# jmhb0/view_neti

Hardware: AMD Instinct MI355X
Metric: TI train steps/sec (SD-1.5 512^2 bs=4 per GPU) (higher is better)
Workload: dtype f16; 1 GPU; learnable_mode 0, sd15 shapes, 512x512 fp16, bs=4/GPU, grad_accum 1, full train step (VAE+16xCLIP+UNet fwd/bwd+AdamW); global_batch=4, parallelism=dp1, rccl_ranks=1, hipgraph=True

## Files before the change

include/vneti.h:

```cpp
#ifndef VNETI_H
#define VNETI_H
#include <stddef.h>
#include <stdint.h>

#ifdef __cplusplus
extern "C" {
#endif

#define VNETI_ABI_VERSION 1

int vneti_version(void);
int vneti_precision(void);
int vneti_last_error(char* buf, size_t n);

typedef struct vneti_gemm_desc {
  const void* A;
  const void* B;
  void* C;
  long long lda, ldb, ldc;
  int M, N, K;
  int batch;
  long long strideA, strideB, strideC;
  const float* bias;
  const void* rowadd;
// ... 1 lines not shown
  int rows_per_group;
  const void* resid;
  long long ldr;
  float alpha;
  int act;
  int out_f32;
  int conv_mode;
  int Hi, Wi, Ci, Ho, Wo, stride, pad_t, pad_l, ups;
  long long ldx;
  int tile_hint;
  void* workspace;
  long long workspace_bytes;
  int split_k;
  const void* gate_src;
  long long ld_gate;
  int gate_act;
  void* C2;
  long long ldc2;
  int act2;
  void* gn_sums;
  int gn_hw, gn_cpg, gn_groups, gn_slots;
  int geglu;
  int conv_korder;
} vneti_gemm_desc;

int vneti_gemm_f16(const vneti_gemm_desc* d, void* stream);
int vneti_gemm_select_tile(int M, int N, int batch);
int vneti_gemm_select_split(int M, int N, int K, int batch, int tile_hint, long long workspace_bytes);

int vneti_im2col3x3_small(const void* x, int x_is_f32, long long sb, long long sc, long long sy,
                          long long sx, void* out, int Bn, int C, int Hi, int Wi, int Ho, int Wo,
                          int stride, int pad_t, int pad_l, void* stream);

int vneti_conv3x3_in(const void* x, int x_is_f32, long long sb, long long sc, long long sy, long long sx,
                     const void* w_packed, const float* bias, void* out, long long ldo, int Bn, int C, int H, int W,
                     int Co, void* gn_sums, int gn_groups, int gn_slots, void* stream);

int vneti_transpose_f16(const void* in, long long ld_in, long long stride_in, void* out,
                        long long ld_out, long long stride_out, int rows, int cols, int batch,
                        void* stream);
#define VNETI_TRANSPOSE_MAX 4
typedef struct vneti_transpose_desc {
  const void* inp;
  long long ld_in, stride_in;
  void* out;
  long long ld_out, stride_out;
// ... 227 lines not shown
```

view_neti_amd/csrc/gemm_args.h:

```cpp
#pragma once
#include "common.h"

namespace {

struct GemmArgs {
  const half_t* A;
  const half_t* B;
  void* C;
  const float* bias;
  const half_t* rowadd;
  const void* resid;
  float* ws;
  const half_t* gate_src;
  half_t* C2;
  long long ld_gate, ldc2;
  int gate_act, act2;
  float* gn_sums;
  int gn_hw, gn_cpg, gn_G, gn_slots;
  int geglu;
  long long lda, ldb, ldc, ld_rowadd, ldr;
  long long strideA, strideB, strideC;
  uint32_t a_bytes, b_bytes;
  int M, N, K;
  int rows_per_group;
  float alpha;
  int act;
  int out_f32;
  int batch, ksplit, kt_per_split;
  int conv_mode;
  int Hi, Wi, Ci, Ho, Wo, stride, pad_t, pad_l, ups;
  int ldx2;
  int korder;
  int tiles_m, tiles_n;
};

__device__ __forceinline__ float apply_act(float v, int act) {
  switch (act) {
    case 1: return vn_silu(v);
    case 2: return vn_quick_gelu(v);
    case 3: return vn_gelu_erf(v);
    default: return v;
  }
}
__device__ __forceinline__ float act_grad(float f, int act) {
  if (act == 2) {
    float s = vn_sigmoid(1.702f * f);
    return s * (1.f + 1.702f * f * (1.f - s));
  } else if (act == 3) {
    return vn_gelu_erf_grad(f);
  }
  float s = vn_sigmoid(f);
  return s * (1.f + f * (1.f - s));
}

__device__ __forceinline__ int lds_off(int row, int chunk) {
// ... 15 lines not shown
```

view_neti_amd/csrc/gemm_conv.hip:

```cpp
#include "common.h"
#include "gemm_args.h"
#include "../../include/vneti.h"

namespace {

template <int BM, int BN, int WM, int WN, bool F32OUT, bool DMA, int NSTG = 2, int EPI = 2, bool CONV = true>
__global__ __launch_bounds__((BM / WM) * (BN / WN) * 64) void gemm_kernel(
    const half_t* pA, const half_t* pB, uint32_t p_a_bytes, uint32_t p_b_bytes, int p_lda, int p_ldb, int pM, int pN, int pK,
    int p_tiles_m, int p_tiles_n, int p_split_conv , const GemmArgs gfull) {
  GemmArgs g = gfull;
  g.A = pA;
  g.B = pB;
  g.a_bytes = p_a_bytes;
  g.b_bytes = p_b_bytes;
  g.lda = p_lda;
  g.ldb = p_ldb;
  g.M = pM;
  g.N = pN;
  g.K = pK;
  g.tiles_m = p_tiles_m;
  g.tiles_n = p_tiles_n;
  g.kt_per_split = p_split_conv & 0xffff;
  g.ksplit = (p_split_conv >> 16) & 0xff;
  g.conv_mode = p_split_conv >> 24;
// ... 18 lines not shown
  __shared__ __attribute__((aligned(16))) char smem[LDS_BYTES + GN_BYTES];

  const int tid = threadIdx.x;
  const int lane = tid & 63;
  const int wave = __builtin_amdgcn_readfirstlane(tid >> 6);
  const int wm0 = (wave / NWN) * WM;
  const int wn0 = (wave % NWN) * WN;

  int nblk = g.tiles_m * g.tiles_n;
  int bid = blockIdx.x;
  {
    int q = nblk >> 3, r = nblk & 7, xcd = bid & 7, idx = bid >> 3;
    bid = (xcd < r ? xcd * (q + 1) : r * (q + 1) + (xcd - r) * q) + idx;
  }
  const int tile_m = bid / g.tiles_n;
  const int tile_n = bid - tile_m * g.tiles_n;
  const int m0 = tile_m * BM;
  const int n0 = tile_n * BN;
  const int bz = blockIdx.y;
  const int kz = blockIdx.z;

  const half_t* Ab = g.A + (long long)bz * g.strideA;
  const half_t* Bb = g.B + (long long)bz * g.strideB;
  __amdgpu_buffer_rsrc_t rsA = vn_make_rsrc(Ab, g.a_bytes);
  __amdgpu_buffer_rsrc_t rsB = vn_make_rsrc(Bb, g.b_bytes);

  const int lrow = tid >> 3;
  const int gchunk = DMA ? ((tid & 7) ^ ((lrow >> 1) & 7)) : (tid & 7);

  const float rcp_hw = CONV ? __builtin_amdgcn_rcpf((float)(g.Ho * g.Wo)) : 0.f, rcp_wo = CONV ? __builtin_amdgcn_rcpf((float)g.Wo) : 0.f;
  int a_off[A_IT];
  int a_py[A_IT], a_px[A_IT], a_bh[A_IT];
#pragma unroll
  for (int i = 0; i < A_IT; ++i) {
    int m = m0 + lrow + RSTEP * i;
    bool ok = m < g.M;
    if (e_conv == 0) {
      a_off[i] = ok ? (int)((long long)m * g.lda * 2) + gchunk * 16 : -1;
      a_py[i] = a_px[i] = a_bh[i] = 0;
    } else {
      int rem, ox;
      const int b = vn_divmod(m, g.Ho * g.Wo, rcp_hw, rem);
      const int oy = vn_divmod(rem, g.Wo, rcp_wo, ox);
      a_bh[i] = ok ? b * g.Hi : -1;
      if (e_conv == 1) {
        a_py[i] = oy * g.stride - g.pad_t;
        a_px[i] = ox * g.stride - g.pad_l;
      } else {
        a_py[i] = oy + g.pad_t;
        a_px[i] = ox + g.pad_l;
      }
      a_off[i] = ((b * g.Hi + a_py[i]) * g.Wi + a_px[i]) * g.ldx2 + gchunk * 16;
    }
  }
  int b_off[B_IT];
#pragma unroll
  for (int i = 0; i < B_IT; ++i) {
    int n = n0 + lrow + RSTEP * i;
    b_off[i] = (n < g.N) ? (int)((long long)n * g.ldb * 2) + gchunk * 16 : -1;
  }

  u32x4 ra[DMA ? 1 : A_IT], rb[DMA ? 1 : B_IT];

  auto a_offset = [&](int i, int k0, int dy, int dx, int tapoff) -> uint32_t {
    if (e_conv == 0) return a_off[i] < 0 ? VN_OOB : (uint32_t)(a_off[i] + k0 * 2);
    bool ok = a_bh[i] >= 0;
    if (e_conv == 1 && !g.ups) {
      int iy = a_py[i] + dy, ix = a_px[i] + dx;
      ok = ok && (unsigned)iy < (unsigned)g.Hi && (unsigned)ix < (unsigned)g.Wi;
      return ok ? (uint32_t)(a_off[i] + tapoff) : VN_OOB;
    }
    int iy, ix;
    if (e_conv == 1) {
      iy = a_py[i] + dy;
      ix = a_px[i] + dx;
      ok = ok && (unsigned)iy < (unsigned)(2 * g.Hi) && (unsigned)ix < (unsigned)(2 * g.Wi);
      iy >>= 1;
      ix >>= 1;
    } else {
      int ty = a_py[i] - dy, tx = a_px[i] - dx;
      ok = ok && ty >= 0 && tx >= 0;
      if (g.stride == 2) {
        ok = ok && ((ty | tx) & 1) == 0;
        ty >>= 1;
        tx >>= 1;
      }
      iy = ty;
      ix = tx;
      ok = ok && iy < g.Hi && ix < g.Wi;
    }
    return ok ? (uint32_t)(((a_bh[i] + iy) * g.Wi + ix) * g.ldx2 + tapoff) : VN_OOB;
  };

  uint32_t a_cur[A_IT], b_cur[B_IT];
#pragma unroll
  for (int i = 0; i < B_IT; ++i) b_cur[i] = b_off[i] < 0 ? VN_OOB : (uint32_t)b_off[i];

  auto issue = [&](int kt, int stage, bool first) {
    const int k0 = kt * 64;
    bool recompute = first;
    int dy = 0, dx = 0, tapoff = 0;
    if (e_conv != 0) {
      int tap, ci0;
      if (g.korder) {
        const int chunk = kt / 9;
        tap = kt - chunk * 9;
        ci0 = chunk << 6;
        recompute = true;
      } else {
        tap = k0 / g.Ci;
        ci0 = k0 - tap * g.Ci;
        recompute = recompute || ci0 == 0;
      }
      if (recompute) {
        dy = tap / 3;
        dx = tap - dy * 3;
        tapoff = (e_conv == 1 && !g.ups) ? ((dy * g.Wi + dx) * g.ldx2 + ci0 * 2) : (ci0 * 2 + gchunk * 16);
      }
    }
    if (recompute) {
#pragma unroll
      for (int i = 0; i < A_IT; ++i) a_cur[i] = a_offset(i, k0, dy, dx, tapoff);
      if (first) {
#pragma unroll
        for (int i = 0; i < B_IT; ++i) b_cur[i] += (uint32_t)k0 * 2;
      }
    }
    if constexpr (DMA) {
      char* As = smem + stage * STAGE_BYTES;
      char* Bs = As + BM * 128;
#pragma unroll
      for (int i = 0; i < A_IT; ++i) dma16(rsA, As + (wave * 8 + RSTEP * i) * 128, a_cur[i]);
#pragma unroll
      for (int i = 0; i < B_IT; ++i) dma16(rsB, Bs + (wave * 8 + RSTEP * i) * 128, b_cur[i]);
    } else {
#pragma unroll
      for (int i = 0; i < A_IT; ++i) ra[i] = vn_buf_load16(rsA, a_cur[i]);
#pragma unroll
      for (int i = 0; i < B_IT; ++i) rb[i] = vn_buf_load16(rsB, b_cur[i]);
    }
// ... 238 lines not shown
        }
      }
      if (gn_img >= 0 && (!uni || lane < CPR)) {
        vn_u64* a = gacc + ((gn_img - gn_img0) * GN_NG + (gn_glo - gn_g0t)) * 4;
        vn_fx_add2(a, s_lo, q_lo);
        if (gn_split < 8) vn_fx_add2(a + 4, s_hi, q_hi);
      }
      s_lo = q_lo = s_hi = q_hi = 0.f;
    };
    for (int idx = tid; idx < BM * CPR; idx += NT) {
      int r = idx / CPR, c = (idx - r * CPR) * 8;
      int m = m0 + r, n = n0 + c;
      const bool valid = m < g.M && n < g.N;
      if (gn) {
        int gn_rem;
        const int img = valid ? vn_divmod(m, g.gn_hw, rcp_gnhw, gn_rem) : gn_img;
        if (__any(img != gn_img)) {
          gn_flush();
          gn_img = img;
        }
      }
      if (!valid) continue;
      half8 v = as_half8(*reinterpret_cast<const u32x4*>(smem + ((size_t)r * CS_LD + c) * 2));
      int ra_rem;
      const half_t* radd = e_rowadd ? e_rowadd + (long long)vn_divmod(m, g.rows_per_group, rcp_rpg, ra_rem) * g.ld_rowadd + n : nullptr;
      if (n + 8 <= g.N) {
        if (radd) {
          half8 t = *reinterpret_cast<const half8*>(radd);
          v = vn_add8(v, t);
        }
        if (Rb) {
          half8 rr = *reinterpret_cast<const half8*>(Rb + (long long)m * g.ldr + n);
          v = vn_add8(v, rr);
        }
        if (e_geglu == 2) {
          const half_t* pp = e_gate + (long long)m * g.ld_gate + 2 * n;
#pragma unroll
          for (int c2 = 0; c2 < 2; ++c2) {
            const half8 pre = *reinterpret_cast<const half8*>(pp + 8 * c2);
            half8 o;
#pragma unroll
            for (int e = 0; e < 4; ++e) {
              const float d = (float)v[4 * c2 + e], hh = (float)pre[e], gg = (float)pre[4 + e];
              float cdf, xpdf;
              vn_gelu_parts(gg, cdf, xpdf);
              o[e] = (half_t)(d * gg * cdf);
              o[4 + e] = (half_t)(d * hh * (cdf + xpdf));
            }
            vn_st16_wt(rsC, (uint32_t)(((long long)m * g.ldc + 2 * n + 8 * c2) * 2), o);
          }
          continue;
        }
        if (e_gate) {
          half8 pre = *reinterpret_cast<const half8*>(e_gate + (long long)m * g.ld_gate + n);
#pragma unroll
          for (int e = 0; e < 8; ++e) v[e] = (half_t)((float)v[e] * act_grad((float)pre[e], g.gate_act));
        }
        if (e_geglu == 1 || (e_C2 && e_geglu == 0)) vn_st16_wt_saved(rsC, (uint32_t)(((long long)m * g.ldc + n) * 2), v);
        else vn_st16_wt(rsC, (uint32_t)(((long long)m * g.ldc + n) * 2), v);
        if (e_geglu == 1) {
          half4 o2;
#pragma unroll
          for (int e = 0; e < 4; ++e) o2[e] = (half_t)((float)v[e] * vn_gelu_erf((float)v[4 + e]));
          *reinterpret_cast<half4*>(e_C2 + (long long)m * g.ldc2 + (n >> 1)) = o2;
        }
        if (gn) {
#pragma unroll
          for (int e = 0; e < 8; ++e) {
            const float x = (float)v[e];
            if (e < gn_split) {
              s_lo += x;
              q_lo += x * x;
            } else {
              s_hi += x;
              q_hi += x * x;
            }
          }
        }
        if (e_C2 && e_geglu == 0) {
          half8 o2;
#pragma unroll
          for (int e = 0; e < 8; ++e) o2[e] = (half_t)apply_act((float)v[e], g.act2);
          vn_st16_wt(rsC2, (uint32_t)(((long long)m * g.ldc2 + n) * 2), o2);
        }
      } else {
        for (int e = 0; e < 8 && n + e < g.N; ++e) {
          float x = (float)v[e];
          if (radd) x = (float)(half_t)(x + (float)radd[e]);
          if (Rb) x = (float)(half_t)(x + (float)Rb[(long long)m * g.ldr + n + e]);
          if (e_gate) x = (float)(half_t)(x * act_grad((float)e_gate[(long long)m * g.ld_gate + n + e], g.gate_act));
          Cb[(long long)m * g.ldc + n + e] = (half_t)x;
          if (e_C2) e_C2[(long long)m * g.ldc2 + n + e] = (half_t)apply_act((float)(half_t)x, g.act2);
          if (gn) {
            const float xs = (float)(half_t)x;
            if (e < gn_split) {
              s_lo += xs;
              q_lo += xs * xs;
            } else {
              s_hi += xs;
              q_hi += xs * xs;
            }
          }
        }
      }
    }
    if (gn) {
      gn_flush();
      __syncthreads();
      const int slot = tile_m % g.gn_slots;
      for (int i = tid; i < GN_IMG * GN_NG; i += NT) {
        const vn_u64* src = gacc + 4 * i;
        if ((src[0] | src[1] | src[2] | src[3]) == 0) continue;
        const int img = gn_img0 + i / GN_NG, grp = gn_g0t + i % GN_NG;
        vn_u64* dst = reinterpret_cast<vn_u64*>(e_gn_sums) + (((long long)img * g.gn_slots + slot) * g.gn_G + grp) * 4;
// ... 244 lines not shown
  g.geglu = d->geglu;
  g.lda = d->lda;
  g.ldb = d->ldb;
  g.ldc = d->ldc;
  g.ld_rowadd = d->ld_rowadd;
  g.ldr = d->ldr;
  g.strideA = d->strideA;
  g.strideB = d->strideB;
  g.strideC = d->strideC;
  g.M = d->M;
  g.N = d->N;
  g.K = d->K;
  g.batch = batch;
  g.rows_per_group = d->rows_per_group > 0 ? d->rows_per_group : 1;
  g.alpha = d->alpha;
  g.act = d->act;
  g.out_f32 = d->out_f32 ? 1 : 0;
  g.conv_mode = d->conv_mode;
  long long a_bytes;
  if (d->conv_mode == 0) {
    VN_REQUIRE(d->lda % 8 == 0, "gemm: lda=%lld must be a multiple of 8", d->lda);
    a_bytes = ((long long)(d->M - 1) * d->lda + d->K) * 2;
  } else {
    VN_REQUIRE(d->conv_mode == 1 || d->conv_mode == 2, "gemm: bad conv_mode %d", d->conv_mode);
    VN_REQUIRE(d->Ci > 0 && d->Ci % 64 == 0, "conv: Ci=%d must be a multiple of 64", d->Ci);
    VN_REQUIRE(d->K == 9 * d->Ci, "conv: K=%d must equal 9*Ci=%d", d->K, 9 * d->Ci);
    VN_REQUIRE(d->stride == 1 || d->stride == 2, "conv: stride %d unsupported", d->stride);
    VN_REQUIRE(d->Ho > 0 && d->Wo > 0 && d->M % (d->Ho * d->Wo) == 0, "conv: M=%d not a multiple of Ho*Wo", d->M);
    VN_REQUIRE(d->ldx % 8 == 0, "conv: ldx must be a multiple of 8");
    VN_REQUIRE(!(d->ups && d->conv_mode != 1), "conv: fused upsample only in forward gather mode");
    VN_REQUIRE(!(d->ups && d->stride != 1), "conv: fused upsample needs stride 1");
    g.Hi = d->Hi;
    g.Wi = d->Wi;
    g.Ci = d->Ci;
    g.Ho = d->Ho;
    g.Wo = d->Wo;
    g.stride = d->stride;
    g.pad_t = d->pad_t;
    g.pad_l = d->pad_l;
    g.ups = d->ups;
    g.ldx2 = (int)(d->ldx * 2);
    VN_REQUIRE(!d->conv_korder || d->Ci % 64 == 0, "conv: conv_korder=1 needs Ci=%d to be a multiple of 64", d->Ci);
    g.korder = d->conv_korder ? 1 : 0;
    long long nb = d->M / (d->Ho * d->Wo);
    a_bytes = nb * d->Hi * d->Wi * d->ldx * 2;
  }
  long long b_bytes = ((long long)(d->N - 1) * d->ldb + d->K) * 2;
  VN_REQUIRE(a_bytes < 0x7fffffffLL && b_bytes < 0x7fffffffLL, "gemm: operand larger than 2 GiB");
  g.a_bytes = (uint32_t)a_bytes;
  g.b_bytes = (uint32_t)b_bytes;
  if (!d->out_f32) {
    VN_REQUIRE(d->ldc % 8 == 0 || d->N < 8, "gemm: ldc=%lld must be a multiple of 8", d->ldc);
  }
  VN_REQUIRE_OUT("gemm C", vn_out_bytes(d->M, d->ldc, d->N, d->out_f32 ? 4 : 2, batch, d->strideC));
  if (d->C2) VN_REQUIRE_OUT("gemm C2", vn_out_bytes(d->M, d->ldc2, d->geglu == 1 ? d->N / 2 : d->N, 2));
  hipStream_t st = (hipStream_t)stream;
  bool f32 = d->out_f32 != 0;
  VN_REQUIRE(!(f32 && d->rowadd), "gemm: rowadd is only supported for f16 output");
  if (d->gate_src || d->C2) {
    VN_REQUIRE(!f32 && batch == 1, "gemm: gate/C2 epilogues need f16 output and batch 1");
    VN_REQUIRE(!d->gate_src || (d->gate_act >= 1 && d->gate_act <= 3 && d->ld_gate % 8 == 0), "gemm: bad gate arguments");
    VN_REQUIRE(!d->C2 || (d->act2 >= 0 && d->act2 <= 3 && d->ldc2 % 8 == 0), "gemm: bad C2 arguments");
  }

  if (d->geglu) {
    VN_REQUIRE(d->geglu == 1 || d->geglu == 2, "gemm: geglu must be 0, 1 or 2");
    VN_REQUIRE(!f32 && batch == 1 && d->N % 8 == 0, "gemm: geglu needs f16 output, batch 1 and N %% 8 == 0");
    VN_REQUIRE(d->split_k == 1, "gemm: geglu needs split_k = 1 (it lives in the fused epilogue)");
    VN_REQUIRE(!d->gn_sums, "gemm: geglu and gn_sums are exclusive");
    if (d->geglu == 1) {
      VN_REQUIRE(d->C2 && d->ldc2 % 4 == 0 && !d->gate_src, "gemm: geglu forward needs C2 ([M][N/2]) and no gate");
    } else {
      VN_REQUIRE(d->gate_src && d->ld_gate % 8 == 0 && !d->C2 && !d->resid && !d->rowadd,
                 "gemm: geglu backward needs gate_src ([M][2N] saved pre-activation) and a plain epilogue");
      VN_REQUIRE(d->ldc % 8 == 0, "gemm: geglu backward writes [M][2N]: ldc %% 8");
    }
  }
  if (d->gn_sums) {
    VN_REQUIRE(!f32 && batch == 1, "gemm: gn_sums needs f16 output and batch 1");
    VN_REQUIRE(d->gn_hw >= 64 && d->gn_cpg >= 4 && d->gn_groups > 0 && d->gn_slots > 0 && d->N == d->gn_cpg * d->gn_groups &&
                   d->M % d->gn_hw == 0 && (d->gn_cpg >= 8 || d->gn_cpg == 4),
               "gemm: bad gn_sums geometry hw=%d cpg=%d G=%d", d->gn_hw, d->gn_cpg, d->gn_groups);
    VN_REQUIRE(d->split_k == 1, "gemm: gn_sums needs split_k = 1 (the statistics live in the fused epilogue)");
  }

  int cfg = d->tile_hint;
  bool dma = true;
  if (cfg >= 100) {
    dma = false;
    cfg -= 100;
  }
  if (cfg == 0) cfg = select_tile(d->M, d->N, batch);
  VN_REQUIRE(cfg >= 1 && cfg <= kMaxTile, "gemm: unknown tile_hint %d", d->tile_hint);
  if (cfg == 18 &&
      (d->conv_mode < 1 || d->conv_mode > 2 || d->stride != 1 || d->ups || d->pad_t != 1 || d->pad_l != 1 || d->Hi != d->Ho ||
       d->Wi != d->Wo || (d->Ho & 15) || (d->Wo & 15) || (d->Ci & 63) || !d->conv_korder || batch != 1 || f32))
    cfg = 17;
  if (cfg == 18 && d->gn_sums && (d->gn_cpg & 1)) cfg = 17;
  if ((cfg == 16 || cfg == 17) && (!dma || (d->conv_mode && (d->ups || (d->conv_mode == 2 && d->stride == 2))) ||
                    (d->gn_sums && (d->gn_cpg & 1)) ||
                    (d->M >= (1 << 24) && (d->conv_mode || d->rowadd || d->gn_sums)))) cfg = cfg == 16 ? 5 : 7;
  if ((cfg == 5 || cfg == 16) && f32) cfg = 4;
  if (cfg == 17 && f32) cfg = 7;
  if ((cfg == 6 || cfg == 7) && !dma) cfg = 4;
  if (cfg >= 10 && !dma) cfg = kTiles[cfg].bm == 128 ? (kTiles[cfg].bn == 128 ? 1 : 2) : 3;
  long long ws_floats = d->workspace ? d->workspace_bytes / 4 : 0;
  int ks = d->split_k;
  if (ks == 0) ks = select_ksplit(d->M, d->N, d->K, batch, cfg, ws_floats);
  if (ks < 1) ks = 1;
  const int nk = d->K / 64;
  if (ks > nk) ks = nk;
  if (ks > 1) {
    VN_REQUIRE(d->workspace && (long long)ks * batch * d->M * d->N <= ws_floats,
               "gemm: split_k=%d needs %lld workspace bytes", ks, (long long)ks * batch * d->M * d->N * 4);
    VN_REQUIRE(batch == 1 || (d->strideC != 0), "gemm: batched split-K needs strideC");
    VN_REQUIRE((long long)batch * d->M * ((d->N + 3) / 4) < 0x7fffffffLL, "gemm: split-K output larger than 2^31 chunks");
    VN_REQUIRE_OUT("gemm split-K workspace", (long long)ks * batch * d->M * d->N * 4);
  }
  if (cfg == 18 && ks > d->Ci / 64) ks = d->Ci / 64;
  g.ksplit = ks;
  g.kt_per_split = cdiv(nk, ks);
  g.ksplit = cdiv(nk, g.kt_per_split);
// ... 34 lines not shown
```

view_neti_amd/engine/schedule.py:

```python
from __future__ import annotations

from functools import partial
from typing import Dict, List

import torch

from .. import lib, ops, packing


class T:

    __slots__ = ("v", "g", "gw", "rows", "cols", "children", "need_grad", "producer")

    def __init__(self, v, g=None, need_grad=True):
        self.v = v
        self.g = g
        self.gw = False
        self.rows, self.cols = v.shape
        self.children: List["T"] = []
        self.need_grad = need_grad
        self.producer = None


def rup(x, m):
# ... 51 lines not shown
    def _grad(self, t: T):
        if t.g is None:
            t.g = self._buf((t.rows, t.cols))
        return t.g

    def _contrib(self, t: T, fn, extra=None):
        g = self._grad(t)
        if t.gw:
            if extra is not None:
                self.bwd.append(partial(ops.add, g, extra, g))
            self.bwd.append(self._tagged(partial(fn, g, g), fn))
        else:
            self.bwd.append(self._tagged(partial(fn, g, extra), fn))
            t.gw = True
            for c in t.children:
                c.gw = True

    @staticmethod
    def _tagged(p, fn):
        if hasattr(fn, "vn_cost"):
            p.vn_cost = fn.vn_cost
        return p

    def _contrib_gemm(self, t: T, A, Bm, **kw):
        g = self._grad(t)
        resid = g if t.gw else None
        self.bwd.append(partial(ops.gemm, A, Bm, g, resid=resid, **kw))
        if not t.gw:
            t.gw = True
            for c in t.children:
                c.gw = True

    _tile_cache: Dict[tuple, int] = {}
    _TILE_DIMS = {1: (128, 128), 2: (128, 64), 3: (64, 64), 4: (256, 128), 5: (256, 256), 6: (256, 128), 7: (256, 128),
                  8: (256, 128), 9: (128, 128), 10: (128, 128), 11: (128, 64), 12: (64, 64), 13: (128, 128), 14: (128, 64),
                  15: (64, 64), 16: (256, 256), 17: (256, 128), 18: (256, 128)}

    @staticmethod
    def _gemm_key(f):
        kw = f.keywords
        A, Bm, out = f.args[:3]
        conv = kw.get("conv")
        M = kw.get("M") or A.shape[-2]
        N = kw.get("N") or Bm.shape[-2]
        K = kw.get("K") or Bm.shape[-1]
        ck = (conv["mode"], conv["stride"], conv["ups"], conv["Hi"], conv["Wi"]) if conv else None
        return (M, N, K, kw.get("batch") or 1, ck, out.dtype == torch.float32, kw.get("geglu") or 0)

    def autotune(self, candidates=(1, 2, 3, 5, 6, 7, 8, 9, 10, 11, 12, 13, 14, 15, 16, 17, 18), reps=8):
        if not torch.cuda.is_available():
# ... 44 lines not shown
            t = _time_call(partial(ops.gemm, *args, **kw), args[0], *how)
            if t < best_t:
                best, best_t = (h, sk, ko), t
        return best, B_cm

    def _pin(self, f, pick, B_cm=None):
        pick = tuple(pick) + (0,) * (3 - len(pick))
        conv = f.keywords.get("conv")
        kw = dict(f.keywords)
        kw["tile_hint"], kw["split_k"] = pick[0], pick[1]
        args = f.args
        if pick[2] and _chunk_major_ok(conv):
            if B_cm is None:
                B_cm = packing._chunk_major(f.args[1], f.args[1].shape[0], conv["Ci"])
            kw["conv"] = dict(conv, korder=1)
            self.bytes += B_cm.numel() * B_cm.element_size()
            args = (f.args[0], B_cm) + tuple(f.args[2:])
        return partial(ops.gemm, *args, **kw)

    def bind_workspace(self):
        for lst in (self.fwd_pre, self.fwd, self.bwd):
            for idx, f in enumerate(lst):
                fn = getattr(f, "func", None)
                if fn is ops.gemm or fn is ops.attn_bwd_dkv:
                    lst[idx] = self._rebound(f, fn, dict(f.keywords, workspace=self.ws))

    @staticmethod
    def _rebound(f, fn, kw):
        return partial(fn, *f.args, **kw)

    GN_SLOTS = 8

    def _produced(self, t: T):
        t.producer = len(self.fwd) - 1
        return t

    GN2_MAX = 512

    def _gn2_slice(self):
        if not hasattr(self, "_gn2_arena"):
            self._gn2_arena = self._buf((self.GN2_MAX, self.B, self.GN_SLOTS, self.groups, 4), torch.int64, zero=True)
            self._gn2_used = 0
        assert self._gn2_used < self.GN2_MAX
        self._gn2_used += 1
        return self._gn2_arena[self._gn2_used - 1]

    def fuse_gn_stats(self, fuse: bool = True):
# ... 146 lines not shown
            self._contrib(x, self._gn_bwd_fn(r["gn1"], dn1), extra=dout)

    def _ln(self, xv, name, w):
        rows, Cc = xv.shape
        rec = dict(x=xv, gamma=self._w32(w[name + ".weight"]), beta=self._w32(w[name + ".bias"]),
                   mean=self._buf((rows,), torch.float32), rstd=self._buf((rows,), torch.float32))
        y = self._buf((rows, Cc))
        self.fwd.append(partial(ops.layernorm_fwd, xv, y, rec["gamma"], rec["beta"], rec["mean"], rec["rstd"], 1e-5))
        return y, rec

    def _ln_bwd(self, rec, dy, dx, accum, f16_copy=None):
        ops.layernorm_bwd(dy, rec["x"], rec["gamma"], rec["mean"], rec["rstd"], dx, accum=accum, f16_copy=f16_copy)

    def _downsample(self, x: T, Cc, name, w, out_view, h, wd, pad=1):
        M = x.rows // 4
        wf = self._w16(packing.conv3x3_fwd(w[name + "weight"]))
        b = self._w32(w[name + "bias"])
        out = T(out_view if out_view is not None else self._buf((M, Cc)))
        self.fwd.append(partial(ops.gemm, x.v, wf, out.v, bias=b, M=M,
                                conv=self._conv_desc(h, wd, Cc, h // 2, wd // 2, 2, pad, 0, x.v.stride(0))))
        self._produced(out)
        rec = dict(kind="down", x=x, out=out, C=Cc, h=h, wd=wd, pad=pad)
        if self.need_backward:
            rec["wd_"] = self._w16(packing.conv3x3_dgrad(w[name + "weight"]))
        self.tape.append(rec)
        return out

    def _downsample_bwd(self, r):
        x, out, Cc, h, wd = r["x"], r["out"], r["C"], r["h"], r["wd"]
        assert out.gw
        desc = self._conv_desc(h // 2, wd // 2, Cc, h, wd, 2, r["pad"], 0, out.g.stride(0), mode=2)
        self._contrib_gemm(x, out.g, r["wd_"], M=x.rows, conv=desc)

    def forward_pre(self):
        for f in self.fwd_pre:
            f()

    def forward_main(self):
        for f in self.fwd:
            f()

    def forward(self):
        self.forward_pre()
        self.forward_main()

    def backward(self):
        for f in self.bwd:
            f()


def _chunk_major_ok(conv) -> bool:
    return bool(conv) and not conv.get("ups") and not conv.get("korder") and \
        not (conv["mode"] == 2 and conv["stride"] == 2) and conv["Ci"] % 64 == 0 and conv["Ci"] >= 128


def gemm_variants(key, conv, geglu, candidates) -> List[tuple]:
    M, N, K, batch = key[:4]
    try_cm = _chunk_major_ok(conv)
    halo_ok = try_cm and conv["mode"] in (1, 2) and conv["stride"] == 1 and conv["pad_t"] == 1 and conv["pad_l"] == 1 \
        and conv["Ho"] % 16 == 0 and conv["Wo"] % 16 == 0 and conv["Hi"] == conv["Ho"] and conv["Wi"] == conv["Wo"]
    tiles_ko = [(h, 0) for h in candidates if h != 18] + \
        ([(h, 1) for h in candidates if h in (16, 17) or (h == 18 and halo_ok)] if try_cm else [])
    out = []
    for h, ko in tiles_ko:
        bm, bn = Schedule._TILE_DIMS[h]
        tiles = -(-M // bm) * -(-N // bn) * batch
        sks = (0, 1) + (tuple(x for x in (2, 3, 4, 6, 8, 12)
                              if x * 8 <= K // 64 and tiles * x <= 1024 and x * batch * M * N <= 16 * 2 ** 20)
                        if tiles < 256 else ())
        if geglu:
            sks = (1,)
# ... 56 lines not shown
```

view_neti_amd/ops.py:

```python
from __future__ import annotations

import ctypes as C

import torch

from . import lib as _l

ACT_NONE, ACT_SILU, ACT_QUICK_GELU, ACT_GELU = 0, 1, 2, 3


def stream() -> int:
    return torch.cuda.current_stream().cuda_stream


def _p(t):
    return None if t is None else t.data_ptr()


def _ld(t):
    if t is None:
        return 0
    assert t.stride(-1) == 1, "last dim must be contiguous"
    return t.stride(-2) if t.dim() >= 2 else t.shape[-1]

# ... 7 lines not shown


def gemm(A, B, out, *, bias=None, rowadd=None, rows_per_group=1, resid=None, alpha=1.0, act=0,
         tile_hint=0, batch=0, strideA=0, strideB=0, strideC=0, M=None, N=None, K=None, conv=None,
         lda=None, ldc=None, workspace=None, split_k=0, gate=None, gate_act=0, out2=None, act2=0,
         gn_sums=None, gn_hw=0, gn_groups=0, gn_slots=0, geglu=0):
    d = _l.GemmDesc()
    d.A, d.B, d.C = _p(A), _p(B), _p(out)
    d.ldb = _ld(B)
    d.ldc = ldc if ldc is not None else _ld(out)
    d.N = N if N is not None else B.shape[-2]
    d.K = K if K is not None else B.shape[-1]
    if conv is None:
        d.M = M if M is not None else A.shape[-2]
        d.lda = lda if lda is not None else _ld(A)
        d.conv_mode = 0
    else:
        d.M = M
        d.lda = 0
        d.conv_mode = conv["mode"]
        for k in ("Hi", "Wi", "Ci", "Ho", "Wo", "stride", "pad_t", "pad_l", "ups", "ldx"):
            setattr(d, k, int(conv.get(k, 0)))
        d.conv_korder = int(conv.get("korder", 0))
    d.batch = batch
    d.strideA, d.strideB, d.strideC = strideA, strideB, strideC
    d.bias = _p(bias)
    d.rowadd = _p(rowadd)
    d.ld_rowadd = _ld(rowadd) if rowadd is not None else 0
    d.rows_per_group = rows_per_group
    d.resid = _p(resid)
    d.ldr = _ld(resid) if resid is not None else 0
    d.alpha = alpha
    d.act = act
    d.out_f32 = 1 if out.dtype == torch.float32 else 0
    d.tile_hint = tile_hint
    if gate is not None:
        d.gate_src, d.ld_gate, d.gate_act = _p(gate), _ld(gate), gate_act
    if out2 is not None:
        d.C2, d.ldc2, d.act2 = _p(out2), _ld(out2), act2
    if gn_sums is not None:
        d.gn_sums, d.gn_hw, d.gn_groups, d.gn_slots = _p(gn_sums), gn_hw, gn_groups, gn_slots
        d.gn_cpg = d.N // gn_groups
    d.geglu = geglu
    ws = workspace if workspace is not None else _default_ws
    if ws is not None:
        d.workspace = ws.data_ptr()
        d.workspace_bytes = ws.numel() * ws.element_size()
    d.split_k = split_k if ws is not None else 1
    _l.call("gemm_f16", C.byref(d), stream())


def im2col3x3_small(x, out, Bn, Cc, Hi, Wi, Ho, Wo, stride, pad_t, pad_l, strides):
    sb, sc, sy, sx = strides
    _l.call("im2col3x3_small", _p(x), 1 if x.dtype == torch.float32 else 0, sb, sc, sy, sx, _p(out),
            Bn, Cc, Hi, Wi, Ho, Wo, stride, pad_t, pad_l, stream())


def conv3x3_in(x, w_packed, bias, out, Bn, Cc, H, W, strides, gn_sums=None, gn_hw=0, gn_groups=0, gn_slots=0):
    sb, sc, sy, sx = strides
    assert gn_sums is None or gn_hw == H * W
    _l.call("conv3x3_in", _p(x), 1 if x.dtype == torch.float32 else 0, sb, sc, sy, sx, _p(w_packed), _p(bias), _p(out),
            _ld(out), Bn, Cc, H, W, w_packed.shape[0], _p(gn_sums), gn_groups, gn_slots, stream())


def transpose(inp, out, rows, cols, batch, ld_in, stride_in, ld_out, stride_out):
    _l.call("transpose_f16", _p(inp), ld_in, stride_in, _p(out), ld_out, stride_out, rows, cols, batch, stream())


def transpose_multi(items):
    arr = (_l.TransposeDesc * len(items))()
    for d, (inp, out, rows, cols, batch, ld_in, stride_in, ld_out, stride_out) in zip(arr, items):
        d.inp, d.ld_in, d.stride_in = _p(inp), ld_in, stride_in
        d.out, d.ld_out, d.stride_out = _p(out), ld_out, stride_out
        d.rows, d.cols, d.batch = rows, cols, batch
# ... 458 lines not shown
```

view_neti_amd/packing.py:

```python
from __future__ import annotations

import os

import torch

KORDER_CM = os.environ.get("VNETI_CONV_KORDER", "0") == "1"


def _chunk_major(m: torch.Tensor, n_out: int, c: int) -> torch.Tensor:
    return m.reshape(n_out, 9, c // 64, 64).permute(0, 2, 1, 3).reshape(n_out, 9 * c).contiguous()


def conv3x3_fwd(w: torch.Tensor, cm=None) -> torch.Tensor:
    co, ci, kh, kw = w.shape
    assert kh == 3 and kw == 3
    m = w.permute(0, 2, 3, 1).reshape(co, 9 * ci).contiguous()
    cm = KORDER_CM if cm is None else cm
    return _chunk_major(m, co, ci) if cm and ci % 64 == 0 else m


def conv3x3_dgrad(w: torch.Tensor, cm=None) -> torch.Tensor:
    co, ci, kh, kw = w.shape
    assert kh == 3 and kw == 3
    m = w.permute(1, 2, 3, 0).reshape(ci, 9 * co).contiguous()
    cm = KORDER_CM if cm is None else cm
    return _chunk_major(m, ci, co) if cm and co % 64 == 0 else m


def pad_rows(w: torch.Tensor, mult: int) -> torch.Tensor:
    k = w.shape[-1]
    kp = (k + mult - 1) // mult * mult
    if kp == k:
        return w.contiguous()
    out = torch.zeros(*w.shape[:-1], kp, dtype=w.dtype, device=w.device)
    out[..., :k] = w
    return out


def geglu_interleave_index(n2: int, device=None) -> torch.Tensor:
    F = n2 // 2
    assert n2 % 8 == 0
    r = torch.arange(n2, device=device)
    q, e = r // 8, r % 8
    return torch.where(e < 4, 4 * q + e, F + 4 * q + e - 4)


def geglu_interleave(w: torch.Tensor) -> torch.Tensor:
    return w[geglu_interleave_index(w.shape[0], w.device)].contiguous()

# ... 13 lines not shown
```

view_neti_amd/roofline.py:

```python
from __future__ import annotations

import torch

from . import ops

import os as _os

_CSRC = _os.path.join(_os.path.dirname(_os.path.abspath(__file__)), "csrc")
MFMA_PEAK_TFLOPS = 2500.0
HBM_PEAK_TBS = 8.0
PF, TB = MFMA_PEAK_TFLOPS, HBM_PEAK_TBS


def kernel_tree_sha() -> str:
    import hashlib
    import os
    here = _CSRC
    files = sorted(os.path.join(here, f) for f in os.listdir(here) if f.endswith((".hip", ".h")))
    files.append(os.path.join(os.path.dirname(os.path.dirname(here)), "include", "vneti.h"))
    h = hashlib.sha256()
    for f in files:
        h.update(os.path.basename(f).encode())
        h.update(open(f, "rb").read())
    return h.hexdigest()[:16]


def gemm_cost(f):
    kw = f.keywords
    A, Bm = f.args[0], f.args[1]
    M = kw.get("M") or A.shape[-2]
    N, K = kw.get("N") or Bm.shape[-2], kw.get("K") or Bm.shape[-1]
    batch = kw.get("batch") or 1
    conv = kw.get("conv")
    a_bytes = (M // (conv["Ho"] * conv["Wo"])) * conv["Hi"] * conv["Wi"] * conv["Ci"] * 2 if conv else M * K * 2 * batch
    out = f.args[2]
    c_cols = N * (2 if kw.get("geglu") == 2 else 1)
    extra = sum(M * c * 2 for c, key in ((N, "resid"), (N, "out2"), (c_cols, "gate")) if kw.get(key) is not None)
    if kw.get("geglu") == 1:
        extra -= M * N
    nbytes = a_bytes + N * K * 2 * batch + M * c_cols * out.element_size() * batch + extra
    flops = 2.0 * M * N * K * batch
    return M, N, K, batch, flops, nbytes, flops / (MFMA_PEAK_TFLOPS * 1e12), nbytes / (HBM_PEAK_TBS * 1e12)



def cost(f):
    fn, a, kw = getattr(f, "func", None), getattr(f, "args", ()), getattr(f, "keywords", {}) or {}
    if fn is ops.gemm:
        M, N, K, batch, flops, nbytes, t_mfma, t_hbm = gemm_cost(f)
        if t_hbm > t_mfma:
            return ("gemm, below the ridge (short-K linears: HBM-bound)", 0, nbytes)
        return ("gemm / implicit-GEMM conv (MFMA-bound)", flops, 0)
    if fn in (ops.attn_fwd, ops.attn_bwd_dq, ops.attn_bwd_dkv):
        i = {ops.attn_fwd: 5, ops.attn_bwd_dq: 7, ops.attn_bwd_dkv: 8}[fn]
        Bn, H, Nq, Nk, D = a[i:i + 5]
        causal = a[i + 6]
        mm = {ops.attn_fwd: 2, ops.attn_bwd_dq: 3, ops.attn_bwd_dkv: 4}[fn]
        name = {ops.attn_fwd: "attention fwd", ops.attn_bwd_dq: "attention bwd dQ", ops.attn_bwd_dkv: "attention bwd dK/dV"}[fn]
        scores = Bn * H * Nq * Nk * (0.5 if causal else 1.0)
        ks, db = -(-D // 16), -(-D // 32)
        mfma_c = {ops.attn_fwd: ks + 2 * db, ops.attn_bwd_dq: 2 * ks + 2 * db, ops.attn_bwd_dkv: 2 * ks + 4 * db}[fn] * 32 / 1024.0
        valu_c = {ops.attn_fwd: 2.8, ops.attn_bwd_dq: 4.0, ops.attn_bwd_dkv: 4.0}[fn] * 2 / 64.0 + (2 * 5 / 3) / 64.0
        cob = scores * (mfma_c + valu_c) / (1024 * 2.4e9)
        return (name, mm * 2.0 * scores * D, 0, cob)
    if fn is ops.attn_bwd_small:
        Bn, H, N, D = a[9:13]
        return ("attention bwd (short sequences, one launch)", 7 * 2.0 * Bn * H * N * N * D * (0.5 if a[14] else 1.0), 0)
    if fn in (ops.groupnorm_fwd, ops.groupnorm_fwd_sums, ops.groupnorm_fwd_2l):
        Bn, HW, C = (a[7], a[8], a[9]) if fn is ops.groupnorm_fwd else (a[8], a[9], a[10])
        return ("GroupNorm(+SiLU) fwd" + (" (stats in producer)" if fn is ops.groupnorm_fwd_sums else ""), 0, 2.0 * Bn * HW * C * 2)
    if fn is ops.layernorm_fwd:
# ... 85 lines not shown
```

Baseline: 38.44 steps/s.

## Use sub-pixel phase decomposition for stride-2 downsample conv data-gradient

Replaces the stride-2 3x3 conv dgrad (a full 9-tap gather over zero-inserted positions) with a phase-decomposed conv. Each of the four output parity phases runs as one slot of a batch-4 GEMM using only its 1, 2 or 4 taps, and the epilogue scatters rows back to interleaved positions. This removes the multiply-by-zero work and wasted gathers of the 9-tap formulation. In exchange it uses a new conv_mode with packed tap words, forces split_k=1, and gives up the specialized DMA and cfg16/17/18 tiles, so tile choice could reduce efficiency.

```diff
diff --git a/include/vneti.h b/include/vneti.h
--- a/include/vneti.h
+++ b/include/vneti.h
@@ -47,6 +47,8 @@
   int gn_hw, gn_cpg, gn_groups, gn_slots;
   int geglu;
   int conv_korder;
+  int ph_ntaps0, ph_ntaps1, ph_ntaps2, ph_ntaps3;
+  unsigned ph_taps0, ph_taps1, ph_taps2, ph_taps3;
 } vneti_gemm_desc;
 
 int vneti_gemm_f16(const vneti_gemm_desc* d, void* stream);
diff --git a/view_neti_amd/csrc/gemm_args.h b/view_neti_amd/csrc/gemm_args.h
--- a/view_neti_amd/csrc/gemm_args.h
+++ b/view_neti_amd/csrc/gemm_args.h
@@ -31,6 +31,7 @@
   int Hi, Wi, Ci, Ho, Wo, stride, pad_t, pad_l, ups;
   int ldx2;
   int korder;
+  uint32_t ph_ntaps, ph_taps0, ph_taps1, ph_taps2, ph_taps3;
   int tiles_m, tiles_n;
 };
 
diff --git a/view_neti_amd/csrc/gemm_conv.hip b/view_neti_amd/csrc/gemm_conv.hip
--- a/view_neti_amd/csrc/gemm_conv.hip
+++ b/view_neti_amd/csrc/gemm_conv.hip
@@ -64,6 +64,17 @@
 
   const half_t* Ab = g.A + (long long)bz * g.strideA;
   const half_t* Bb = g.B + (long long)bz * g.strideB;
+  uint32_t ph_tp = 0;
+  if (e_conv == 3) {
+    int before = 0;
+#pragma unroll
+    for (int p = 0; p < 3; ++p) before += p < bz ? (int)((g.ph_ntaps >> (4 * p)) & 15u) : 0;
+    const int ntaps = (int)((g.ph_ntaps >> (4 * bz)) & 15u);
+    ph_tp = bz == 0 ? g.ph_taps0 : bz == 1 ? g.ph_taps1 : bz == 2 ? g.ph_taps2 : g.ph_taps3;
+    Bb = g.B + before * g.Ci;
+    g.K = ntaps * g.Ci;
+    g.b_bytes -= (uint32_t)(before * g.Ci) * 2u;
+  }
   __amdgpu_buffer_rsrc_t rsA = vn_make_rsrc(Ab, g.a_bytes);
   __amdgpu_buffer_rsrc_t rsB = vn_make_rsrc(Bb, g.b_bytes);
 
@@ -85,7 +96,7 @@
       const int b = vn_divmod(m, g.Ho * g.Wo, rcp_hw, rem);
       const int oy = vn_divmod(rem, g.Wo, rcp_wo, ox);
       a_bh[i] = ok ? b * g.Hi : -1;
-      if (e_conv == 1) {
+      if (e_conv != 2) {
         a_py[i] = oy * g.stride - g.pad_t;
         a_px[i] = ox * g.stride - g.pad_l;
       } else {
@@ -107,13 +118,13 @@
   auto a_offset = [&](int i, int k0, int dy, int dx, int tapoff) -> uint32_t {
     if (e_conv == 0) return a_off[i] < 0 ? VN_OOB : (uint32_t)(a_off[i] + k0 * 2);
     bool ok = a_bh[i] >= 0;
-    if (e_conv == 1 && !g.ups) {
+    if (e_conv != 2 && !g.ups) {
       int iy = a_py[i] + dy, ix = a_px[i] + dx;
       ok = ok && (unsigned)iy < (unsigned)g.Hi && (unsigned)ix < (unsigned)g.Wi;
       return ok ? (uint32_t)(a_off[i] + tapoff) : VN_OOB;
     }
     int iy, ix;
-    if (e_conv == 1) {
+    if (e_conv != 2) {
       iy = a_py[i] + dy;
       ix = a_px[i] + dx;
       ok = ok && (unsigned)iy < (unsigned)(2 * g.Hi) && (unsigned)ix < (unsigned)(2 * g.Wi);
@@ -155,9 +166,15 @@
         recompute = recompute || ci0 == 0;
       }
       if (recompute) {
-        dy = tap / 3;
-        dx = tap - dy * 3;
-        tapoff = (e_conv == 1 && !g.ups) ? ((dy * g.Wi + dx) * g.ldx2 + ci0 * 2) : (ci0 * 2 + gchunk * 16);
+        if (e_conv == 3) {
+          const uint32_t t = ph_tp >> (8 * tap);
+          dy = (int)((t >> 4) & 15u) - 8;
+          dx = (int)(t & 15u) - 8;
+        } else {
+          dy = tap / 3;
+          dx = tap - dy * 3;
+        }
+        tapoff = (e_conv != 2 && !g.ups) ? ((dy * g.Wi + dx) * g.ldx2 + ci0 * 2) : (ci0 * 2 + gchunk * 16);
       }
     }
     if (recompute) {
@@ -442,6 +459,13 @@
       }
       if (!valid) continue;
       half8 v = as_half8(*reinterpret_cast<const u32x4*>(smem + ((size_t)r * CS_LD + c) * 2));
+      int mo = m;
+      if (e_conv == 3) {
+        int prem, px_;
+        const int pb = vn_divmod(m, g.Ho * g.Wo, rcp_hw, prem);
+        const int py_ = vn_divmod(prem, g.Wo, rcp_wo, px_);
+        mo = ((pb * 2 * g.Ho + 2 * py_ + (bz >> 1)) * 2 * g.Wo) + 2 * px_ + (bz & 1);
+      }
       int ra_rem;
       const half_t* radd = e_rowadd ? e_rowadd + (long long)vn_divmod(m, g.rows_per_group, rcp_rpg, ra_rem) * g.ld_rowadd + n : nullptr;
       if (n + 8 <= g.N) {
@@ -450,7 +474,7 @@
           v = vn_add8(v, t);
         }
         if (Rb) {
-          half8 rr = *reinterpret_cast<const half8*>(Rb + (long long)m * g.ldr + n);
+          half8 rr = *reinterpret_cast<const half8*>(Rb + (long long)mo * g.ldr + n);
           v = vn_add8(v, rr);
         }
         if (e_geglu == 2) {
@@ -467,7 +491,7 @@
               o[e] = (half_t)(d * gg * cdf);
               o[4 + e] = (half_t)(d * hh * (cdf + xpdf));
             }
-            vn_st16_wt(rsC, (uint32_t)(((long long)m * g.ldc + 2 * n + 8 * c2) * 2), o);
+            vn_st16_wt(rsC, (uint32_t)(((long long)mo * g.ldc + 2 * n + 8 * c2) * 2), o);
           }
           continue;
         }
@@ -476,8 +500,8 @@
 #pragma unroll
           for (int e = 0; e < 8; ++e) v[e] = (half_t)((float)v[e] * act_grad((float)pre[e], g.gate_act));
         }
-        if (e_geglu == 1 || (e_C2 && e_geglu == 0)) vn_st16_wt_saved(rsC, (uint32_t)(((long long)m * g.ldc + n) * 2), v);
-        else vn_st16_wt(rsC, (uint32_t)(((long long)m * g.ldc + n) * 2), v);
+        if (e_geglu == 1 || (e_C2 && e_geglu == 0)) vn_st16_wt_saved(rsC, (uint32_t)(((long long)mo * g.ldc + n) * 2), v);
+        else vn_st16_wt(rsC, (uint32_t)(((long long)mo * g.ldc + n) * 2), v);
         if (e_geglu == 1) {
           half4 o2;
 #pragma unroll
@@ -507,9 +531,9 @@
         for (int e = 0; e < 8 && n + e < g.N; ++e) {
           float x = (float)v[e];
           if (radd) x = (float)(half_t)(x + (float)radd[e]);
-          if (Rb) x = (float)(half_t)(x + (float)Rb[(long long)m * g.ldr + n + e]);
+          if (Rb) x = (float)(half_t)(x + (float)Rb[(long long)mo * g.ldr + n + e]);
           if (e_gate) x = (float)(half_t)(x * act_grad((float)e_gate[(long long)m * g.ld_gate + n + e], g.gate_act));
-          Cb[(long long)m * g.ldc + n + e] = (half_t)x;
+          Cb[(long long)mo * g.ldc + n + e] = (half_t)x;
           if (e_C2) e_C2[(long long)m * g.ldc2 + n + e] = (half_t)apply_act((float)(half_t)x, g.act2);
           if (gn) {
             const float xs = (float)(half_t)x;
@@ -800,10 +824,36 @@
     VN_REQUIRE(d->lda % 8 == 0, "gemm: lda=%lld must be a multiple of 8", d->lda);
     a_bytes = ((long long)(d->M - 1) * d->lda + d->K) * 2;
   } else {
-    VN_REQUIRE(d->conv_mode == 1 || d->conv_mode == 2, "gemm: bad conv_mode %d", d->conv_mode);
+    VN_REQUIRE(d->conv_mode >= 1 && d->conv_mode <= 3, "gemm: bad conv_mode %d", d->conv_mode);
     VN_REQUIRE(d->Ci > 0 && d->Ci % 64 == 0, "conv: Ci=%d must be a multiple of 64", d->Ci);
-    VN_REQUIRE(d->K == 9 * d->Ci, "conv: K=%d must equal 9*Ci=%d", d->K, 9 * d->Ci);
-    VN_REQUIRE(d->stride == 1 || d->stride == 2, "conv: stride %d unsupported", d->stride);
+    if (d->conv_mode == 3) {
+      VN_REQUIRE(d->batch <= 1, "phase conv: the batch slot carries the phase");
+      VN_REQUIRE(!d->out_f32 && !d->rowadd && !d->gate_src && !d->C2 && !d->geglu && !d->gn_sums,
+                 "phase conv: f16 output with bias / resid only");
+      VN_REQUIRE(d->split_k == 1, "phase conv needs split_k = 1");
+      VN_REQUIRE(d->Hi == d->Ho && d->Wi == d->Wo && !d->ups && !d->conv_korder,
+                 "phase conv: Hi x Wi = Ho x Wo source grid, tap-major K, no ups");
+      const int nt[4] = {d->ph_ntaps0, d->ph_ntaps1, d->ph_ntaps2, d->ph_ntaps3};
+      const unsigned tp[4] = {d->ph_taps0, d->ph_taps1, d->ph_taps2, d->ph_taps3};
+      int ntmax = 0;
+      for (int p = 0; p < 4; ++p) {
+        VN_REQUIRE(nt[p] >= 1 && nt[p] <= 4, "phase conv: phase %d has %d taps (1..4)", p, nt[p]);
+        VN_REQUIRE(nt[p] == 4 || (tp[p] >> (8 * nt[p])) == 0, "phase conv: phase %d lists more than its %d taps", p, nt[p]);
+        if (nt[p] > ntmax) ntmax = nt[p];
+        g.ph_ntaps |= (uint32_t)nt[p] << (4 * p);
+      }
+      VN_REQUIRE(d->K == ntmax * d->Ci, "phase conv: K=%d must equal max taps * Ci=%d", d->K, ntmax * d->Ci);
+      g.ph_taps0 = tp[0];
+      g.ph_taps1 = tp[1];
+      g.ph_taps2 = tp[2];
+      g.ph_taps3 = tp[3];
+      batch = 4;
+      g.batch = 4;
+      g.strideA = g.strideB = g.strideC = 0;
+    } else {
+      VN_REQUIRE(d->K == 9 * d->Ci, "conv: K=%d must equal 9*Ci=%d", d->K, 9 * d->Ci);
+    }
+    VN_REQUIRE(d->stride == 1 || d->stride == 2 || d->conv_mode == 3, "conv: stride %d unsupported", d->stride);
     VN_REQUIRE(d->Ho > 0 && d->Wo > 0 && d->M % (d->Ho * d->Wo) == 0, "conv: M=%d not a multiple of Ho*Wo", d->M);
     VN_REQUIRE(d->ldx % 8 == 0, "conv: ldx must be a multiple of 8");
     VN_REQUIRE(!(d->ups && d->conv_mode != 1), "conv: fused upsample only in forward gather mode");
@@ -813,9 +863,9 @@
     g.Ci = d->Ci;
     g.Ho = d->Ho;
     g.Wo = d->Wo;
-    g.stride = d->stride;
-    g.pad_t = d->pad_t;
-    g.pad_l = d->pad_l;
+    g.stride = d->conv_mode == 3 ? 1 : d->stride;
+    g.pad_t = d->conv_mode == 3 ? 0 : d->pad_t;
+    g.pad_l = d->conv_mode == 3 ? 0 : d->pad_l;
     g.ups = d->ups;
     g.ldx2 = (int)(d->ldx * 2);
     VN_REQUIRE(!d->conv_korder || d->Ci % 64 == 0, "conv: conv_korder=1 needs Ci=%d to be a multiple of 64", d->Ci);
@@ -823,14 +873,18 @@
     long long nb = d->M / (d->Ho * d->Wo);
     a_bytes = nb * d->Hi * d->Wi * d->ldx * 2;
   }
-  long long b_bytes = ((long long)(d->N - 1) * d->ldb + d->K) * 2;
+  long long b_cols = d->K;
+  if (d->conv_mode == 3) b_cols = (long long)(d->ph_ntaps0 + d->ph_ntaps1 + d->ph_ntaps2 + d->ph_ntaps3) * d->Ci;
+  VN_REQUIRE(d->conv_mode != 3 || d->ldb >= b_cols, "phase conv: ldb=%lld is shorter than the four phases' %lld columns", d->ldb, b_cols);
+  long long b_bytes = ((long long)(d->N - 1) * d->ldb + b_cols) * 2;
   VN_REQUIRE(a_bytes < 0x7fffffffLL && b_bytes < 0x7fffffffLL, "gemm: operand larger than 2 GiB");
   g.a_bytes = (uint32_t)a_bytes;
   g.b_bytes = (uint32_t)b_bytes;
   if (!d->out_f32) {
     VN_REQUIRE(d->ldc % 8 == 0 || d->N < 8, "gemm: ldc=%lld must be a multiple of 8", d->ldc);
   }
-  VN_REQUIRE_OUT("gemm C", vn_out_bytes(d->M, d->ldc, d->N, d->out_f32 ? 4 : 2, batch, d->strideC));
+  if (d->conv_mode == 3) VN_REQUIRE_OUT("gemm C", vn_out_bytes(4LL * d->M, d->ldc, d->N, 2));
+  else VN_REQUIRE_OUT("gemm C", vn_out_bytes(d->M, d->ldc, d->N, d->out_f32 ? 4 : 2, batch, d->strideC));
   if (d->C2) VN_REQUIRE_OUT("gemm C2", vn_out_bytes(d->M, d->ldc2, d->geglu == 1 ? d->N / 2 : d->N, 2));
   hipStream_t st = (hipStream_t)stream;
   bool f32 = d->out_f32 != 0;
@@ -870,12 +924,13 @@
   }
   if (cfg == 0) cfg = select_tile(d->M, d->N, batch);
   VN_REQUIRE(cfg >= 1 && cfg <= kMaxTile, "gemm: unknown tile_hint %d", d->tile_hint);
+  const bool generic_conv = d->conv_mode == 3;
   if (cfg == 18 &&
-      (d->conv_mode < 1 || d->conv_mode > 2 || d->stride != 1 || d->ups || d->pad_t != 1 || d->pad_l != 1 || d->Hi != d->Ho ||
+      (generic_conv || d->conv_mode < 1 || d->conv_mode > 2 || d->stride != 1 || d->ups || d->pad_t != 1 || d->pad_l != 1 || d->Hi != d->Ho ||
        d->Wi != d->Wo || (d->Ho & 15) || (d->Wo & 15) || (d->Ci & 63) || !d->conv_korder || batch != 1 || f32))
     cfg = 17;
   if (cfg == 18 && d->gn_sums && (d->gn_cpg & 1)) cfg = 17;
-  if ((cfg == 16 || cfg == 17) && (!dma || (d->conv_mode && (d->ups || (d->conv_mode == 2 && d->stride == 2))) ||
+  if ((cfg == 16 || cfg == 17) && (!dma || generic_conv || (d->conv_mode && (d->ups || (d->conv_mode == 2 && d->stride == 2))) ||
                     (d->gn_sums && (d->gn_cpg & 1)) ||
                     (d->M >= (1 << 24) && (d->conv_mode || d->rowadd || d->gn_sums)))) cfg = cfg == 16 ? 5 : 7;
   if ((cfg == 5 || cfg == 16) && f32) cfg = 4;
diff --git a/view_neti_amd/engine/schedule.py b/view_neti_amd/engine/schedule.py
--- a/view_neti_amd/engine/schedule.py
+++ b/view_neti_amd/engine/schedule.py
@@ -97,10 +97,10 @@
             p.vn_cost = fn.vn_cost
         return p
 
-    def _contrib_gemm(self, t: T, A, Bm, **kw):
+    def _contrib_gemm(self, t: T, A, Bm, launcher=ops.gemm, **kw):
         g = self._grad(t)
         resid = g if t.gw else None
-        self.bwd.append(partial(ops.gemm, A, Bm, g, resid=resid, **kw))
+        self.bwd.append(partial(launcher, A, Bm, g, resid=resid, **kw))
         if not t.gw:
             t.gw = True
             for c in t.children:
@@ -191,7 +191,7 @@
         for lst in (self.fwd_pre, self.fwd, self.bwd):
             for idx, f in enumerate(lst):
                 fn = getattr(f, "func", None)
-                if fn is ops.gemm or fn is ops.attn_bwd_dkv:
+                if fn in ops.GEMM_LAUNCHERS or fn is ops.attn_bwd_dkv:
                     lst[idx] = self._rebound(f, fn, dict(f.keywords, workspace=self.ws))
 
     @staticmethod
@@ -384,15 +384,26 @@
         self._produced(out)
         rec = dict(kind="down", x=x, out=out, C=Cc, h=h, wd=wd, pad=pad)
         if self.need_backward:
-            rec["wd_"] = self._w16(packing.conv3x3_dgrad(w[name + "weight"]))
+            if pad == 1 and phase_dgrad_ok(Cc):
+                Bm, rec["wd_kw"] = packing.conv3x3_s2_dgrad_phases(w[name + "weight"])
+                rec["wd_"] = self._w16(Bm)
+            else:
+                rec["wd_"] = self._w16(packing.conv3x3_dgrad(w[name + "weight"]))
         self.tape.append(rec)
         return out
 
     def _downsample_bwd(self, r):
         x, out, Cc, h, wd = r["x"], r["out"], r["C"], r["h"], r["wd"]
         assert out.gw
-        desc = self._conv_desc(h // 2, wd // 2, Cc, h, wd, 2, r["pad"], 0, out.g.stride(0), mode=2)
-        self._contrib_gemm(x, out.g, r["wd_"], M=x.rows, conv=desc)
+        if "wd_kw" not in r:
+            desc = self._conv_desc(h // 2, wd // 2, Cc, h, wd, 2, r["pad"], 0, out.g.stride(0), mode=2)
+            self._contrib_gemm(x, out.g, r["wd_"], M=x.rows, conv=desc)
+            return
+        M = x.rows // 4
+        conv = dict(mode=3, Hi=h // 2, Wi=wd // 2, Ci=Cc, Ho=h // 2, Wo=wd // 2, stride=1, pad_t=0, pad_l=0, ups=0,
+                    ldx=out.g.stride(0), **r["wd_kw"])
+        self._contrib_gemm(x, out.g, r["wd_"], M=M, N=Cc, K=4 * Cc, conv=conv, launcher=ops.conv_resample,
+                           **phase_dgrad_pick(M, Cc, 4 * Cc))
 
     def forward_pre(self):
         for f in self.fwd_pre:
@@ -409,6 +420,21 @@
     def backward(self):
         for f in self.bwd:
             f()
+
+
+PHASE_DGRAD_TILES = {
+    (4096, 320, 1280): 7,
+}
+PHASE_DGRAD_MAX_KTILES = 64
+
+
+def phase_dgrad_ok(C: int) -> bool:
+    return C % 64 == 0 and 9 * C // 64 < PHASE_DGRAD_MAX_KTILES
+
+
+def phase_dgrad_pick(M: int, N: int, K: int) -> Dict[str, int]:
+    tile = PHASE_DGRAD_TILES.get((M, N, K)) or ops.gemm_select_tile(M, N, 4)
+    return dict(tile_hint=tile, split_k=1)
 
 
 def _chunk_major_ok(conv) -> bool:
diff --git a/view_neti_amd/ops.py b/view_neti_amd/ops.py
--- a/view_neti_amd/ops.py
+++ b/view_neti_amd/ops.py
@@ -53,6 +53,10 @@
         for k in ("Hi", "Wi", "Ci", "Ho", "Wo", "stride", "pad_t", "pad_l", "ups", "ldx"):
             setattr(d, k, int(conv.get(k, 0)))
         d.conv_korder = int(conv.get("korder", 0))
+        if d.conv_mode == 3:
+            for p in range(4):
+                setattr(d, f"ph_ntaps{p}", int(conv["ph_ntaps"][p]))
+                setattr(d, f"ph_taps{p}", int(conv["ph_taps"][p]))
     d.batch = batch
     d.strideA, d.strideB, d.strideC = strideA, strideB, strideC
     d.bias = _p(bias)
@@ -81,6 +85,13 @@
     _l.call("gemm_f16", C.byref(d), stream())
 
 
+def conv_resample(A, B, out, **kw):
+    gemm(A, B, out, **kw)
+
+
+GEMM_LAUNCHERS = (gemm, conv_resample)
+
+
 def im2col3x3_small(x, out, Bn, Cc, Hi, Wi, Ho, Wo, stride, pad_t, pad_l, strides):
     sb, sc, sy, sx = strides
     _l.call("im2col3x3_small", _p(x), 1 if x.dtype == torch.float32 else 0, sb, sc, sy, sx, _p(out),
diff --git a/view_neti_amd/packing.py b/view_neti_amd/packing.py
--- a/view_neti_amd/packing.py
+++ b/view_neti_amd/packing.py
@@ -25,6 +25,31 @@
     m = w.permute(1, 2, 3, 0).reshape(ci, 9 * co).contiguous()
     cm = KORDER_CM if cm is None else cm
     return _chunk_major(m, ci, co) if cm and co % 64 == 0 else m
+
+
+_STRIDE2_DGRAD_AXIS = (((0, (1,)),), ((1, (0,)), (0, (2,))))
+
+
+def _phase_pack(wk: torch.Tensor, axis):
+    cols, ntaps, words = [], [], []
+    for py in (0, 1):
+        for px in (0, 1):
+            word, t = 0, 0
+            for oy, dys in axis[py]:
+                for ox, dxs in axis[px]:
+                    (dy,), (dx,) = dys, dxs
+                    cols.append(wk[:, :, dy, dx])
+                    word |= (((oy + 8) << 4) | (ox + 8)) << (8 * t)
+                    t += 1
+            ntaps.append(t)
+            words.append(word)
+    return torch.cat(cols, 1).contiguous(), dict(ph_ntaps=tuple(ntaps), ph_taps=tuple(words))
+
+
+def conv3x3_s2_dgrad_phases(w: torch.Tensor):
+    co, ci, kh, kw = w.shape
+    assert kh == 3 and kw == 3
+    return _phase_pack(w.transpose(0, 1), _STRIDE2_DGRAD_AXIS)
 
 
 def pad_rows(w: torch.Tensor, mult: int) -> torch.Tensor:
diff --git a/view_neti_amd/roofline.py b/view_neti_amd/roofline.py
--- a/view_neti_amd/roofline.py
+++ b/view_neti_amd/roofline.py
@@ -40,13 +40,17 @@
         extra -= M * N
     nbytes = a_bytes + N * K * 2 * batch + M * c_cols * out.element_size() * batch + extra
     flops = 2.0 * M * N * K * batch
+    if conv and conv["mode"] == 3:
+        taps = sum(conv["ph_ntaps"])
+        nbytes = a_bytes + N * taps * conv["Ci"] * 2 + 4 * M * N * 2 * (2 if kw.get("resid") is not None else 1)
+        flops = 2.0 * M * N * taps * conv["Ci"]
     return M, N, K, batch, flops, nbytes, flops / (MFMA_PEAK_TFLOPS * 1e12), nbytes / (HBM_PEAK_TBS * 1e12)
 
 
 
 def cost(f):
     fn, a, kw = getattr(f, "func", None), getattr(f, "args", ()), getattr(f, "keywords", {}) or {}
-    if fn is ops.gemm:
+    if fn in ops.GEMM_LAUNCHERS:
         M, N, K, batch, flops, nbytes, t_mfma, t_hbm = gemm_cost(f)
         if t_hbm > t_mfma:
             return ("gemm, below the ridge (short-K linears: HBM-bound)", 0, nbytes)
```

New measurement: 38.52 steps/s, median of 6. No clear change (+0.2%).
